# crowsonkb/k-diffusion

Hardware: AMD Instinct MI355X
Metric: images/sec, 256x256 image_transformer_v2, 50-step DPM++2M (whole job) (higher is better)
Workload: dtype f32

## Files before the change

### include/kdiff_hip.h

```cpp
#ifndef KDIFF_HIP_H
#define KDIFF_HIP_H

#ifdef __cplusplus
extern "C" {
#endif

#define KD_OK 0
#define KD_EINVAL (-1)
#define KD_ELAUNCH (-2)

int kd_version(void);
const char* kd_last_error(void);
int kd_set_option(const char* name, int value);
int kd_get_option(const char* name, int dflt);

enum { KD_A_PLAIN = 0, KD_A_MERGE2x2 = 1, KD_A_PATCH_NCHW = 2 };
enum { KD_PREC_EXACT = 0, KD_PREC_SPLIT3 = 1,
       KD_PREC_BF16 = 2  };
enum { KD_EPI_STORE = 0, KD_EPI_RESIDUAL = 1, KD_EPI_GEGLU = 2, KD_EPI_SPLIT_LERP = 3, KD_EPI_UNPATCH_NCHW = 4,
       KD_EPI_QKV = 5  };

typedef struct {
  int M, N, K;
  int a_mode, epi;
// ... 14 lines not shown
  const float* fac;
  int precision;
  const void* Wp;
  int n_heads;
  const float* qk_scale;
  const float* rope_cos;
  const float* rope_sin;
  int qkv_packed;
  const float* rope_pos;
  const float* rope_freq;
  int a_split, c_split;
  const void* A_lo;
  void* C_lo;
  int per_row;
} KdGemm;

int kd_gemm_f32(const KdGemm* desc, void* stream);

int kd_gemm_bf16(const KdGemm* desc, void* stream);
long long kd_packed_weight_bytes_bf16(int N, int K, int geglu);
int kd_pack_weight_bf16(const float* W, void* out, int N, int K, int geglu, void* stream);

typedef struct KdFfn {
  const void* x;
  void* out;
  const float* scale;
  int scale_stride, rows_per_sample;
  float eps;
  const void* Wp_up;
  const void* Wp_down;
  int M, K, d_ff;
  const void* attn;
  const void* Wp_out;
} KdFfn;
int kd_ffn_bf16_supported(int M, int K, int d_ff);
int kd_ffn_bf16(const KdFfn* desc, void* stream);
int kd_ffn_f32_supported(int M, int K, int d_ff);
int kd_ffn_f32(const KdFfn* desc, void* stream);

long long kd_packed_weight_bytes(int N, int K, int geglu);
int kd_pack_weight_bf16x3(const float* W, void* out, int N, int K, int geglu, void* stream);

int kd_norm_split_f32(const float* x, const float* scale, int scale_stride, int rows_per_sample, void* hi, void* lo, int M, int K,
                      float eps, void* stream);

int kd_rmsnorm_f32(const float* x, const float* scale, float* y, int rows, int d, float eps, void* stream);

int kd_fourier_sigma_f32(const float* sigma, const float* weight, float* ff, int batch, int half, void* stream);
int kd_fourier_f32(const float* in, const float* weight, float* ff, int batch, int in_dim, int half, void* stream);
int kd_cond_sum_f32(float* out, const float* a, const float* b, int b_rows, const float* emb,
                    const long long* ids, const float* c, int batch, int d, void* stream);

int kd_qk_prep_f32(float* qkv, const float* scale_h, const float* cos_t, const float* sin_t,
                   int batch, int tokens_per_sample, int nh, float eps, void* stream);

int kd_attn_global_f32(const float* qkv, float* out, int batch, int T, int nh,
                       int prep, const float* scale_h, const float* cos_t, const float* sin_t, float eps,
                       int precision, void* stream);

int kd_attn_window_f32(const float* qkv, float* out, int batch, int H, int W, int nh, int ws, int shift,
                       int prep, const float* scale_h, const float* cos_t, const float* sin_t, float eps,
                       int precision, void* stream);

int kd_attn_na2d_f32(const float* qkv, float* out, int batch, int H, int W, int nh, int ks,
                     int prep, const float* scale_h, const float* cos_t, const float* sin_t, float eps,
                     int precision, void* stream);

int kd_attn_global_bf16(const void* qkv, void* out, int batch, int T, int nh, void* stream);
int kd_attn_window_bf16(const void* qkv, void* out, int batch, int H, int W, int nh, int ws, int shift, void* stream);
int kd_attn_na2d_bf16(const void* qkv, void* out, int batch, int H, int W, int nh, int ks, void* stream);
// ... 97 lines not shown
```

### k-diffusion_amd/_native.py

```python
import ctypes as C
import os

_HERE = os.path.dirname(os.path.abspath(__file__))
LIB_PATH = os.environ.get("KDIFF_HIP_LIB") or os.path.join(_HERE, "csrc", "libkdiff_hip.so")

A_PLAIN, A_MERGE2x2, A_PATCH_NCHW = 0, 1, 2
EPI_STORE, EPI_RESIDUAL, EPI_GEGLU, EPI_SPLIT_LERP, EPI_UNPATCH_NCHW, EPI_QKV = 0, 1, 2, 3, 4, 5
PREC_EXACT, PREC_SPLIT3, PREC_BF16 = 0, 1, 2
PC_ONE, PC_SKIP, PC_OUT, PC_IN = 0, 1, 2, 3
PREC_FP8 = 3
_MODES = {"exact": PREC_EXACT, "split3": PREC_SPLIT3, "bf16": PREC_BF16, "fp8": PREC_FP8}


def default_precision():
    mode = os.environ.get("KDIFF_GEMM", "split3").lower()
    if mode not in _MODES:
        raise ValueError(f"KDIFF_GEMM={mode!r}: expected one of {sorted(_MODES)}")
    return _MODES[mode]


def kernel_precision():
    p = default_precision()
    return PREC_BF16 if p == PREC_FP8 else p


def precision_name(p):
    return {v: k for k, v in _MODES.items()}[p]
(STEP_EULER, STEP_HEUN_PRED, STEP_HEUN_CORR, STEP_DPMPP_2M1, STEP_DPMPP_2M2, STEP_ADD_NOISE, STEP_LERP2, STEP_AXPY,
 STEP_EULER_FROM, STEP_AXPBY, STEP_ADD_DIFF, STEP_TO_D) = range(12)


class KdGemm(C.Structure):
    _fields_ = [
        ("M", C.c_int), ("N", C.c_int), ("K", C.c_int),
        ("a_mode", C.c_int), ("epi", C.c_int), ("norm", C.c_int),
        ("rows_per_sample", C.c_int), ("scale_stride", C.c_int),
        ("gh", C.c_int), ("gw", C.c_int), ("ph", C.c_int), ("pw", C.c_int), ("chan", C.c_int),
        ("eps", C.c_float), ("out_add", C.c_float), ("sigma_data", C.c_float),
        ("A", C.c_void_p), ("W", C.c_void_p), ("C", C.c_void_p), ("R", C.c_void_p),
        ("scale", C.c_void_p), ("sigma", C.c_void_p), ("fac", C.c_void_p),
        ("precision", C.c_int), ("Wp", C.c_void_p),
        ("n_heads", C.c_int), ("qk_scale", C.c_void_p), ("rope_cos", C.c_void_p), ("rope_sin", C.c_void_p),
        ("qkv_packed", C.c_int), ("rope_pos", C.c_void_p), ("rope_freq", C.c_void_p),
        ("a_split", C.c_int), ("c_split", C.c_int), ("A_lo", C.c_void_p), ("C_lo", C.c_void_p),
        ("per_row", C.c_int),
    ]


class KdFfn(C.Structure):
    _fields_ = [
        ("x", C.c_void_p), ("out", C.c_void_p), ("scale", C.c_void_p),
        ("scale_stride", C.c_int), ("rows_per_sample", C.c_int), ("eps", C.c_float),
        ("Wp_up", C.c_void_p), ("Wp_down", C.c_void_p),
        ("M", C.c_int), ("K", C.c_int), ("d_ff", C.c_int),
        ("attn", C.c_void_p), ("Wp_out", C.c_void_p),
    ]


class KdCall(C.Structure):
    _fields_ = [("op", C.c_int), ("f", C.c_float), ("p", C.c_void_p * 5), ("i", C.c_int * 8)]


_vp, _i, _f, _ll, _d = C.c_void_p, C.c_int, C.c_float, C.c_longlong, C.c_double

SIGNATURES = {
    "kd_version": [],
    "kd_last_error": [],
    "kd_set_option": [C.c_char_p, _i],
    "kd_get_option": [C.c_char_p, _i],
    "kd_gemm_f32": [C.POINTER(KdGemm), _vp],
    "kd_gemm_bf16": [C.POINTER(KdGemm), _vp],
    "kd_packed_weight_bytes_bf16": [_i, _i, _i],
    "kd_pack_weight_bf16": [_vp, _vp, _i, _i, _i, _vp],
    "kd_ffn_bf16_supported": [_i, _i, _i],
    "kd_ffn_bf16": [_vp, _vp],
    "kd_ffn_f32_supported": [_i, _i, _i],
    "kd_ffn_f32": [_vp, _vp],
    "kd_attn_global_bf16": [_vp, _vp, _i, _i, _i, _vp],
    "kd_attn_window_bf16": [_vp, _vp, _i, _i, _i, _i, _i, _i, _vp],
    "kd_attn_na2d_bf16": [_vp, _vp, _i, _i, _i, _i, _i, _vp],
    "kd_attn_block_bf16_supported": [_i, _i, _i],
    "kd_attn_block_bf16": [C.POINTER(KdGemm), _vp],
    "kd_proj_block_bf16_supported": [_i, _i, _i, _i],
    "kd_proj_block_bf16": [C.POINTER(KdGemm), _vp],
    "kd_packed_weight_bytes_mx8": [_i, _i, _i],
    "kd_pack_weight_mx8": [_vp, _vp, _i, _i, _i, _vp],
    "kd_gemm_mx8_supported": [_i, _i, _i, _i, _i],
    "kd_gemm_mx8": [C.POINTER(KdGemm), _vp],
    "kd_packed_weight_bytes": [_i, _i, _i],
    "kd_pack_weight_bf16x3": [_vp, _vp, _i, _i, _i, _vp],
    "kd_rmsnorm_f32": [_vp, _vp, _vp, _i, _i, _f, _vp],
    "kd_fourier_sigma_f32": [_vp, _vp, _vp, _i, _i, _vp],
    "kd_fourier_f32": [_vp, _vp, _vp, _i, _i, _i, _vp],
    "kd_cond_sum_f32": [_vp, _vp, _vp, _i, _vp, _vp, _vp, _i, _i, _vp],
    "kd_qk_prep_f32": [_vp, _vp, _vp, _vp, _i, _i, _i, _f, _vp],
    "kd_attn_global_f32": [_vp, _vp, _i, _i, _i, _i, _vp, _vp, _vp, _f, _i, _vp],
    "kd_attn_window_f32": [_vp, _vp, _i, _i, _i, _i, _i, _i, _i, _vp, _vp, _vp, _f, _i, _vp],
    "kd_attn_na2d_f32": [_vp, _vp, _i, _i, _i, _i, _i, _i, _vp, _vp, _vp, _f, _i, _vp],
    "kd_sampler_step_f32": [_i, _vp, _vp, _vp, _vp, _vp, _f, _f, _f, _f, _ll, _vp],
    "kd_precond_in_f32": [_vp, _vp, _vp, _f, _i, _ll, _vp],
    "kd_precond_out_f32": [_vp, _vp, _vp, _vp, _f, _i, _ll, _vp],
    "kd_rows_affine_f32": [_vp, _vp, _vp, _vp, _vp, _i, _ll, _vp],
    "kd_sigma_to_t_f32": [_vp, _vp, _vp, _i, _i, _i, _vp],
    "kd_t_to_sigma_f32": [_vp, _vp, _vp, _i, _i, _vp],
    "kd_dpm_eps_f32": [_vp, _vp, _vp, _f, _ll, _vp],
    "kd_dpm_combine_f32": [_vp, _vp, _vp, _vp, _f, _f, _ll, _vp],
    "kd_dpm_error_partials": [],
    "kd_dpm_error_f32": [_vp, _vp, _vp, _f, _f, _ll, _vp, _vp],
    "kd_brownian_f32": [_vp, _vp, _i, _ll, _d, _d, _d, _d, _f, _i, _vp],
# ... 151 lines not shown
```

### k-diffusion_amd/csrc/common.cpp

```cpp
#include "kd_common.h"
#include <atomic>
#include <climits>
#include <mutex>

namespace kd {

static thread_local char g_err[512] = "";
char* err_buf() { return g_err; }

int fail(int code, const char* fmt, ...) {
  va_list ap;
  va_start(ap, fmt);
  vsnprintf(g_err, sizeof(g_err), fmt, ap);
  va_end(ap);
  return code;
}

static std::atomic<bool> g_prof{false};
static std::mutex g_rec_mutex;
static std::vector<ProfRec> g_recs;

bool prof_on() { return g_prof.load(std::memory_order_relaxed); }

static unsigned g_gen = 0;
// ... 11 lines not shown

void prof_end(ProfTicket t, hipStream_t s) {
  std::lock_guard<std::mutex> lock(g_rec_mutex);
  if (t.gen == g_gen && t.idx >= 0 && t.idx < (int)g_recs.size()) (void)hipEventRecord(g_recs[t.idx].e1, s);
}

}

namespace kd {
int cu_count() {
  static std::atomic<int> cache[64];
  int dev = 0;
  (void)hipGetDevice(&dev);
  if (dev < 0 || dev >= 64) dev = 0;
  int n = cache[dev].load(std::memory_order_relaxed);
  if (n <= 0) {
    if (hipDeviceGetAttribute(&n, hipDeviceAttributeMultiprocessorCount, dev) != hipSuccess || n <= 0) n = 256;
    cache[dev].store(n, std::memory_order_relaxed);
  }
  return n;
}
}

using namespace kd;

namespace kd {
namespace {
struct Opt { const char* name; std::atomic<int> value; std::atomic<bool> set; };
Opt g_opts[] = {{"skinny", {0}, {false}}, {"astat", {0}, {false}}, {"ksplit", {0}, {false}}, {"astat_max_k", {0}, {false}}, {"astat_waves", {0}, {false}},
                {"astat_storewait", {0}, {false}}, {"gemm_debug", {0}, {false}}, {"bf16_fast", {0}, {false}}, {"wstat", {0}, {false}},
                {"wstat_waves", {0}, {false}}, {"wstat_max_slices", {0}, {false}}, {"wstat_prefetch", {0}, {false}}, {"astat_bf16", {0}, {false}},
                {"astat_splits", {0}, {false}}, {"tiled_bm", {0}, {false}}, {"attn_global_qw", {0}, {false}},
                {"patch_fast", {0}, {false}}, {"ffn_fused", {0}, {false}}, {"ffn_fused_256", {0}, {false}}, {"astat_rows", {0}, {false}}, {"tiled_deep", {0}, {false}}, {"code_warm", {0}, {false}}, {"ffn_variant", {0}, {false}},
                {"x3", {0}, {false}}, {"x3_splits", {0}, {false}}, {"ffn_x3", {0}, {false}}, {"ffn_x3_half", {0}, {false}}, {"x3_res", {0}, {false}}, {"attn_x3", {0}, {false}}, {"x3_half", {0}, {false}}, {"x3r", {0}, {false}}, {"x3_unpatch", {0}, {false}}, {"x3r_lw", {0}, {false}}, {"x3r_split", {0}, {false}}, {"tiled_lw", {0}, {false}}, {"x3_min_rows", {0}, {false}}, {"x3r_min_rows", {0}, {false}}, {"ffn_x3_min_panels_256", {0}, {false}}, {"x3s_max_rows", {0}, {false}}, {"x3s_max_wgs", {0}, {false}}, {"x3s_scale_lds", {0}, {false}}, {"b16s_max_rows", {0}, {false}}, {"b16s_max_wgs", {0}, {false}}, {"ffn_bf16_min_rows", {0}, {false}}, {"x3s_trace", {0}, {false}}, {"attn_block_bf16", {0}, {false}}, {"proj_block_bf16", {0}, {false}}, {"mx8", {0}, {false}}, {"mx8_splits", {0}, {false}}, {"mx8_min_rows", {0}, {false}}};
constexpr int N_OPTS = sizeof(g_opts) / sizeof(g_opts[0]);
}
int option_index(const char* name) {
  for (int i = 0; i < N_OPTS; ++i)
    if (!strcmp(g_opts[i].name, name)) return i;
  return -1;
}
int option_at(int idx, int dflt) {
  if (idx < 0) return dflt;
  return g_opts[idx].set.load(std::memory_order_relaxed) ? g_opts[idx].value.load(std::memory_order_relaxed) : dflt;
}
}

extern "C" int kd_set_option(const char* name, int value) {
  if (!name) return fail(KD_EINVAL, "kd_set_option: null name");
  const int i = option_index(name);
  if (i < 0) return fail(KD_EINVAL, "kd_set_option: unknown option '%s'", name);
  if (value == INT_MIN) {
    g_opts[i].set.store(false, std::memory_order_relaxed);
    return KD_OK;
  }
  g_opts[i].value.store(value, std::memory_order_relaxed);
  g_opts[i].set.store(true, std::memory_order_relaxed);
  return KD_OK;
}
extern "C" int kd_get_option(const char* name, int dflt) { return name ? option_at(option_index(name), dflt) : dflt; }

extern "C" int kd_version(void) { return 200; }
extern "C" const char* kd_last_error(void) { return err_buf(); }

extern "C" int kd_prof_enable(int on) { g_prof.store(on != 0, std::memory_order_relaxed); return KD_OK; }
extern "C" int kd_prof_count(void) {
  std::lock_guard<std::mutex> lock(g_rec_mutex);
// ... 71 lines not shown
```

### k-diffusion_amd/csrc/ffn_x3.hip

```cpp
#include "x3_common.h"

namespace kd {
namespace x3 {

struct FArgs3 {
  const float* X; float* Y;
  const char* Wu; const char* Wd;
  const float* scale; int scale_stride, rows_per_sample; float eps;
  int M, d_ff, n_tiles;
  int warm;
  unsigned long long* clk;
  const float* Att; const char* Wo;
};

template <int IDX>
__device__ __forceinline__ void mfma_acc_ag(const bf16x8 w, const bf16x8 h) {
  asm volatile("v_mfma_f32_32x32x16_bf16 a[%c2:%c3], %0, %1, a[%c2:%c3]" :: "v"(w), "v"(h), "i"(IDX), "i"(IDX + 15) : KD_AGPR_ALL);
}
template <int IDX>
__device__ __forceinline__ void areg_zero16() {
  static_for<16>([&](auto i_) { asm volatile("v_accvgpr_write_b32 a[%c0], 0" :: "i"(IDX + decltype(i_)::value) : KD_AGPR_ALL); });
}
template <int IDX>
__device__ __forceinline__ f32x4 areg_read4() {
  f32x4 v;
  asm volatile("v_accvgpr_read_b32 %0, a[%c4]\n\tv_accvgpr_read_b32 %1, a[%c5]\n\tv_accvgpr_read_b32 %2, a[%c6]\n\tv_accvgpr_read_b32 %3, a[%c7]"
               : "=v"(v[0]), "=v"(v[1]), "=v"(v[2]), "=v"(v[3]) : "i"(IDX), "i"(IDX + 1), "i"(IDX + 2), "i"(IDX + 3));
  return v;
}

template <int IDX, int BIDX>
__device__ __forceinline__ void mfma_acc_aa(const bf16x8 w) {
  asm volatile("v_mfma_f32_32x32x16_bf16 a[%c1:%c2], %0, a[%c3:%c4], a[%c1:%c2]" :: "v"(w), "i"(IDX), "i"(IDX + 15), "i"(BIDX), "i"(BIDX + 3) : KD_AGPR_ALL);
}

template <int NC , bool OUTP = false >
__global__ __launch_bounds__(256, 1) void ffn_x3_kernel(const FArgs3 p) {
  static_assert(!OUTP || NC == 16, "fused out projection: width 256 here, width 128 in ffn_x3h_kernel");
  constexpr int K = NC * 16, NKU = NC / 2;
  constexpr int NOB = K / 32, NKD = 2 * (K / 128);
  constexpr int UNIT = NKU + NKD;
  constexpr int NSTG = 8, PDIST = NSTG - 1, PB = 4;
  constexpr bool AG = NC >= 16;
  constexpr int AO = AG ? 8 * NC : 0;
  constexpr int WAREA = (NSTG / 4) * STG;
// ... 395 lines not shown
    static_for<4>([&](auto g_) { blk[decltype(g_)::value] = areg_read4<AO + 16 * ob + 4 * decltype(g_)::value>(); });
#pragma unroll
    for (int hb = 0; hb < 2; ++hb) {
      const f32x4 (&skip)[2] = skip_all[ob][hb];
#pragma unroll
      for (int gg = 0; gg < 2; ++gg)
        *reinterpret_cast<f32x4*>(strip + l31 * 64 + (((2 * gg + lh) ^ ((l31 >> 2) & 1)) << 4)) = blk[2 * hb + gg];
#pragma unroll
      for (int it = 0; it < 2; ++it) {
        const int r16 = 16 * it + (lane >> 2), c = lane & 3;
        const f32x4 o = *reinterpret_cast<const f32x4*>(strip + r16 * 64 + ((c ^ ((r16 >> 2) & 1)) << 4));
        if (st_ok[it]) st16(st_row[it] + 32 * ob + 16 * hb, f32x4(o + skip[it]));
      }
    }
  });
  if (probe) { p.clk[2] = __builtin_amdgcn_s_memtime(); p.clk[3] = __builtin_amdgcn_s_memrealtime(); p.clk[7] = (unsigned long long)total; }
  wg_stamp_end(wgs);
}


template <int IDX>
__device__ __forceinline__ void mfma_acc_ag_lo(const bf16x8 w, const bf16x8 h) {
  asm volatile("v_mfma_f32_32x32x16_bf16 a[%c2:%c3], %0, %1, a[%c2:%c3]" :: "v"(w), "v"(h), "i"(IDX), "i"(IDX + 15) : KD_AGPR_LO128);
}
template <int IDX, int BIDX>
__device__ __forceinline__ void mfma_acc_aa_lo(const bf16x8 w) {
  asm volatile("v_mfma_f32_32x32x16_bf16 a[%c1:%c2], %0, a[%c3:%c4], a[%c1:%c2]" :: "v"(w), "i"(IDX), "i"(IDX + 15), "i"(BIDX), "i"(BIDX + 3) : KD_AGPR_LO128);
}
template <int IDX>
__device__ __forceinline__ void areg_zero16_lo() {
  static_for<16>([&](auto i_) { asm volatile("v_accvgpr_write_b32 a[%c0], 0" :: "i"(IDX + decltype(i_)::value) : KD_AGPR_LO128); });
}

template <bool OUTP>
__global__ __launch_bounds__(256, 2) void ffn_x3h_kernel(const FArgs3 p) {
  constexpr int NC = 8, K = 128, NOB = 4;
  constexpr int NSTG = 4, PDIST = NSTG - 1, PB = 4, UNIT = 3;
  constexpr int AO = 64;
  constexpr int CPR = K / 4, PIECES = 32 * CPR / 64, SCL = 1024, SUB = 8192, HALF = 4096;
  extern __shared__ __attribute__((aligned(16))) char smem[];
  const int tid = threadIdx.x, lane = tid & 63, l31 = lane & 31, lh = lane >> 5;
  const int wid = __builtin_amdgcn_readfirstlane(tid >> 6);
  const auto warm = code_warm_begin<16 * 1024>((int)blockIdx.x < p.warm && tid < 64);
  const int m0 = blockIdx.x * 128;
  const int T2 = 2 * p.n_tiles;
  const bool probe = p.clk && blockIdx.x == (gridDim.x * 5) / 8 && tid == 0;
  if (probe) { p.clk[0] = __builtin_amdgcn_s_memtime(); p.clk[1] = __builtin_amdgcn_s_memrealtime(); }
  const WgStamp wgs = wg_stamp_begin(p.clk);

  auto issue_rel = [&](int th, auto off_, int j) {
    constexpr int off = decltype(off_)::value, u = off % UNIT;
    const int tt = min(th + off / UNIT, T2 - 1);
    char* slot = smem + ((th * UNIT + off) % NSTG) * STG;
    const char* src;
    char* dst;
    if constexpr (u < 2) {
      src = p.Wu + ((size_t)(tt >> 1) * (NC / 2) + 2 * u + (j >> 1)) * STG + (j & 1) * IMG + (tt & 1) * HALF + wid * 1024 + lane * 16;
      dst = slot + (j >> 1) * SUB + (j & 1) * HALF + wid * 1024;
    } else {
      src = p.Wd + (size_t)tt * STG + wid * (PB * 1024) + j * 1024 + lane * 16;
      dst = slot + wid * (PB * 1024) + j * 1024;
    }
    __builtin_amdgcn_global_load_lds((const __attribute__((address_space(1))) void*)src, (__attribute__((address_space(3))) void*)dst, 16, 0, 0);
  };

  const int row = m0 + wid * 32 + l31;
  const bool ok = row < p.M;
// ... 328 lines not shown
    const int r = m0 + wid * 32 + 16 * it + (lane >> 2);
    st_ok[it] = r < p.M;
    st_row[it] = p.Y + (size_t)min(r, p.M - 1) * K + 4 * (lane & 3);
    sk_row[it] = p.X + (size_t)min(r, p.M - 1) * K + 4 * (lane & 3);
  }
  f32x4 skip_all[NOB][2][2];
#pragma unroll
  for (int ob = 0; ob < NOB; ++ob)
#pragma unroll
    for (int hb = 0; hb < 2; ++hb)
#pragma unroll
      for (int it = 0; it < 2; ++it)
        skip_all[ob][hb][it] = OUTP ? f32x4{0.f, 0.f, 0.f, 0.f} : *reinterpret_cast<const f32x4*>(sk_row[it] + 32 * ob + 16 * hb);
  __builtin_amdgcn_sched_barrier(0);
  asm volatile("s_waitcnt vmcnt(0)\n\ts_nop 15\n\ts_nop 3" ::: "memory");
  static_for<NOB>([&](auto ob_) {
    constexpr int ob = decltype(ob_)::value;
    f32x4 blk[4];
    static_for<4>([&](auto g_) { blk[decltype(g_)::value] = areg_read4<AO + 16 * ob + 4 * decltype(g_)::value>(); });
#pragma unroll
    for (int hb = 0; hb < 2; ++hb) {
      const f32x4 (&skip)[2] = skip_all[ob][hb];
#pragma unroll
      for (int gg = 0; gg < 2; ++gg)
        *reinterpret_cast<f32x4*>(strip + l31 * 64 + (((2 * gg + lh) ^ ((l31 >> 2) & 1)) << 4)) = blk[2 * hb + gg];
#pragma unroll
      for (int it = 0; it < 2; ++it) {
        const int r16 = 16 * it + (lane >> 2), c = lane & 3;
        const f32x4 o = *reinterpret_cast<const f32x4*>(strip + r16 * 64 + ((c ^ ((r16 >> 2) & 1)) << 4));
        if (st_ok[it]) st16(st_row[it] + 32 * ob + 16 * hb, f32x4(o + skip[it]));
      }
    }
  });
  if (probe) { p.clk[2] = __builtin_amdgcn_s_memtime(); p.clk[3] = __builtin_amdgcn_s_memrealtime(); p.clk[7] = (unsigned long long)(T2 * UNIT); }
  wg_stamp_end(wgs);
}

extern unsigned long long* g_clk;

template <bool OUTP>
static int launch_ffn_half(const FArgs3& a, const char* nm, double flops, double bytes, hipStream_t s) {
  constexpr int LDS = 4 * STG + 4 * 1024 + 4 * 2048;
  auto kern = ffn_x3h_kernel<OUTP>;
  static LdsAttr attr_set;
  attr_set.ensure(reinterpret_cast<const void*>(kern), LDS);
  LaunchScope prof(nm, flops, bytes, s);
  hipLaunchKernelGGL(kern, dim3((unsigned)((a.M + 127) / 128)), dim3(256), LDS, s, a);
  return check_launch("kd_ffn_f32");
}

template <int NC, bool OUTP = false>
static int launch_ffn(const FArgs3& a, const char* nm, double flops, double bytes, hipStream_t s) {
  auto kern = ffn_x3_kernel<NC, OUTP>;
  constexpr int K = NC * 16;
  constexpr int LDS = 8 * STG + 4 * (K * 4 < 1024 ? 1024 : K * 4) + 4 * 2048;
  static LdsAttr attr_set;
  attr_set.ensure(reinterpret_cast<const void*>(kern), LDS);
  LaunchScope prof(nm, flops, bytes, s);
  hipLaunchKernelGGL(kern, dim3((unsigned)((a.M + 127) / 128)), dim3(256), LDS, s, a);
  return check_launch("kd_ffn_f32");
}

}
}

using namespace kd;

extern "C" int kd_ffn_f32_supported(int M, int K, int d_ff) {
  if (!option("ffn_x3", 1)) return 0;
  if (!((K == 128 || K == 256) && d_ff > 0 && d_ff % 64 == 0)) return 0;
  if (K == 128) return M >= 2048;
  int dev = 0, cus = 256;
  (void)hipGetDevice(&dev);
  if (hipDeviceGetAttribute(&cus, hipDeviceAttributeMultiprocessorCount, dev) != hipSuccess || cus <= 0) cus = 256;
  const int need = option("ffn_x3_min_panels_256", cus - cus / 8);
  return (M + 127) / 128 >= need;
}

extern "C" int kd_ffn_f32(const KdFfn* dp, void* stream) {
  if (!dp) return fail(KD_EINVAL, "kd_ffn_f32: null descriptor");
  const KdFfn& d = *dp;
  if (!d.x || !d.out || !d.scale || !d.Wp_up || !d.Wp_down) return fail(KD_EINVAL, "kd_ffn_f32: null x / out / scale / Wp_up / Wp_down");
  if ((d.K != 128 && d.K != 256) || d.d_ff <= 0 || (d.d_ff & 63) || d.M <= 0) return fail(KD_EINVAL, "kd_ffn_f32: K must be 128 or 256, d_ff a multiple of 64 (K=%d d_ff=%d)", d.K, d.d_ff);
  if (d.rows_per_sample <= 0 || (d.scale_stride & 3)) return fail(KD_EINVAL, "kd_ffn_f32: rows_per_sample > 0, scale_stride %% 4 == 0");
  x3::FArgs3 a{};
  a.X = reinterpret_cast<const float*>(d.x); a.Y = reinterpret_cast<float*>(d.out);
  a.Wu = reinterpret_cast<const char*>(d.Wp_up); a.Wd = reinterpret_cast<const char*>(d.Wp_down);
  a.scale = d.scale; a.scale_stride = d.scale_stride; a.rows_per_sample = d.rows_per_sample; a.eps = d.eps;
  a.M = d.M; a.d_ff = d.d_ff; a.n_tiles = d.d_ff / 64;
  a.warm = option("code_warm", KD_CODE_WARM_DEFAULT);
  a.clk = x3::g_clk;
  const double flops = 2.0 * d.M * 3.0 * d.d_ff * d.K;
  const double bytes = 4.0 * (2.0 * d.M * d.K + 3.0 * d.d_ff * d.K);
  char nm[96] = "ffn_x3";
  if (prof_on()) snprintf(nm, sizeof(nm), "ffn_x3 M=%d K=%d d_ff=%d", d.M, d.K, d.d_ff);
  if (d.attn) {
    if (!d.Wp_out) return fail(KD_EINVAL, "kd_ffn_f32: attn without Wp_out");
    a.Att = reinterpret_cast<const float*>(d.attn); a.Wo = reinterpret_cast<const char*>(d.Wp_out);
    const double fl2 = flops + 2.0 * d.M * d.K * d.K, by2 = 4.0 * (3.0 * d.M * d.K + 3.0 * d.d_ff * d.K + (double)d.K * d.K);
    if (prof_on()) snprintf(nm, sizeof(nm), "ffn_x3+out M=%d K=%d d_ff=%d", d.M, d.K, d.d_ff);
    if (d.K == 128) return x3::launch_ffn_half<true>(a, nm, fl2, by2, (hipStream_t)stream);
    return x3::launch_ffn<16, true>(a, nm, fl2, by2, (hipStream_t)stream);
  }
  if (d.K == 128 && option("ffn_x3_half", 1)) return x3::launch_ffn_half<false>(a, nm, flops, bytes, (hipStream_t)stream);
  if (d.K == 128) return x3::launch_ffn<8>(a, nm, flops, bytes, (hipStream_t)stream);
  return x3::launch_ffn<16>(a, nm, flops, bytes, (hipStream_t)stream);
}

KD_TEXT_PAD(ffn_x3)
```

### k-diffusion_amd/models/image_transformer_v2.py

```python
import ctypes as C
import gc
import itertools
import operator
import weakref
import os
import math
from dataclasses import dataclass
from typing import NamedTuple, Optional, Union

import torch
from torch import nn

from .. import _native as nat
from .. import ops
from . import axial_rope

D_HEAD = 64
SCHEDULE_TABLE_MAX_BYTES = 1 << 30
SCHEDULES_KEPT = 4
SCHEDULE_CHAINS_KEPT = 2
DERIVED_KEPT = 1024
MAX_PLANS = 16
PLAN_SWITCHES = (("KDIFF_ATTN_BLOCK", "1"), ("KDIFF_PROJ_BLOCK", "1"), ("KDIFF_FFN_OUT", "all"), ("KDIFF_RUN_LIST", "1"))
CLASS_IDS_KEPT = 4
# ... 323 lines not shown
        self.out_shape = (B, m.out_channels, H, W)
        self.class_checked = {}

        self.sigma = torch.empty(B, **f32)
        self.sigma_ptr = self.sigma.data_ptr()
        self.xs = xs = [torch.empty(B, gh, gw, lv.width, **act) for (gh, gw), lv in zip(grids, levels)]
        self.toks = toks = [B * gh * gw for gh, gw in grids]
        self.qkv = torch.empty(max(t * 3 * lv.width for t, lv in zip(toks, levels)), **act)
        self.att = torch.empty(max(t * lv.width for t, lv in zip(toks, levels)), **act)
        self.hid = torch.empty(max(t * lv.d_ff for t, lv in zip(toks, levels)), **act)
        wide = [t * lv.width for t, lv in zip(toks, levels) if _prepass(mode, lv.width)]
        self.xn = torch.empty(max(wide), **f32) if wide else None
        norm_mods = m._ada_norm_modules()
        self.table_offsets, total = {}, 0
        for name, mod in norm_mods:
            self.table_offsets[name] = 4 * total
            total += mod.linear.weight.shape[0]
        wcat = m._packed.get("ada_norm_wcat")
        if wcat is None or wcat.device != device:
            wcat = m._packed["ada_norm_wcat"] = torch.cat([mod.linear.weight.detach() for _, mod in norm_mods], dim=0).contiguous()
        self.wcat = wcat
        self.scales = [torch.empty(B, total, **f32), torch.empty(B, total, **f32)]
        self.norm_descs = []
        self.last_buf, self.prefetched = 1, None
        self.side_stream = torch.cuda.Stream(device=device)
        self.main_entry = torch.cuda.Event()
        self.schedules, self.schedule_chains = [], {}
        self.scale_width = total
        self.step_chain = self.build_cond(B)

        L = self.launches
        self.d_patch_in = self._gemm(L, "patch_in", None, m.patch_in.proj.weight, xs[0], toks[0], levels[0].width, m.in_channels * ph * pw,
                                     a_mode=nat.A_PATCH_NCHW, grid=grids[0], patch=(ph, pw, m.in_channels))
        for st in hourglass(m):
            li = st.level
            if st.kind == "layer":
                self._add_layer(li, st.prefix, st.module, st.index)
            elif st.kind == "merge":
                self._gemm(L, f"merges.{li}", xs[li], m.merges[li].proj.weight, xs[li + 1], toks[li + 1], levels[li + 1].width,
                           4 * levels[li].width, a_mode=nat.A_MERGE2x2, grid=grids[li + 1])
            else:
                self._gemm(L, f"splits.{li}", xs[li + 1], m.splits[li].proj.weight, xs[li], toks[li + 1], 4 * levels[li].width,
                           levels[li + 1].width, epi=nat.EPI_SPLIT_LERP, residual=xs[li], fac=m.splits[li].fac, grid=grids[li + 1])
        self.d_patch_out = self._gemm(L, "patch_out", xs[0], m.patch_out.proj.weight, None, toks[0], m.out_channels * ph * pw,
                                      levels[0].width, epi=nat.EPI_UNPATCH_NCHW, norm_scale=m.out_norm.scale, scale_stride=0,
                                      rows_per_sample=grids[0][0] * grids[0][1], grid=grids[0], patch=(ph, pw, m.out_channels))
        self._encode_launches()

    def _gemm(self, launches, what, A, Wt, Cc, M, N, K, cond=False, table=None, entry=None, mx8=False, **kw):
        precision = self.cond_precision if cond else self.precision
        if table is not None:
            kw.update(scale_ptr=0, scale_stride=self.scale_width)
        d = ops.gemm(A, Wt, Cc, M=M, N=N, K=K, precision=precision, per_row=cond, mx8=mx8, launch=False, pack=self.model._packed_image, **kw)
        if table is not None:
            self.norm_descs.append((d, self.table_offsets[table]))
        launches.append(_Launch(entry or ops._gemm_entry(precision, mx8), (d,), what + ("(mx8)" if mx8 else "")))
        return d

    def _norm_split(self, launches, table, x, T, d, rps):
        ref = _ScaleRef()
        self.norm_descs.append((ref, self.table_offsets[table]))
        planes = self.xn.view(torch.bfloat16)
        hi, lo = planes[:T * d], planes[T * d:2 * T * d]
        launches.append(_Launch("kd_norm_split_f32", (_ptr(x), ref, self.scale_width, rps, _ptr(hi), _ptr(lo), T, d, 1e-6), table + " (split)"))
        return hi, lo

    def build_cond(self, rows):
        m, f32 = self.model, dict(device=self.device, dtype=torch.float32)
        mw, mdff = m.mapping_spec.width, m.mapping_spec.d_ff
# ... 40 lines not shown

    def _qk(self, li, sa, nh):
        m = self.model
        if self.precision == nat.PREC_BF16:
            cos_t, sin_t = m._rope(li, self.grids, sa, self.device, revs=True)
        else:
            cos_t, sin_t = m._rope(li, self.grids, sa, self.device)
        self.keep += [cos_t, sin_t]
        qk = (sa.scale, cos_t, sin_t, nh)
        if self.precision == nat.PREC_SPLIT3:
            pos_t, freq_t = m._rope(li, self.grids, sa, self.device, revs=True)
            self.keep += [pos_t, freq_t]
            qk += (pos_t, freq_t)
        return qk

    def _add_layer(self, li, prefix, mod, index):
        L, lv, (gh, gw), T = self.launches, self.levels[li], self.grids[li], self.toks[li]
        d, d_ff, x, rps = lv.width, lv.d_ff, self.xs[li], gh * gw
        spec = lv.self_attn
        nh = d // spec.d_head if hasattr(mod, "self_attn") else 0
        kind, core, params = attn_geometry(spec, index) if nh else (None, None, ())
        r = route_layer(self.lib, self.mode, self.B, T, rps, d, d_ff, nh, kind, self.switches)
        split3 = self.precision == nat.PREC_SPLIT3
        if nh:
            sa, norm = mod.self_attn, prefix + "self_attn.norm"
            q = dict(epi=nat.EPI_QKV, rows_per_sample=rps, qk=self._qk(li, sa, nh), qkv_packed=split3)
            if r.qkv == "attn_block":
                self._gemm(L, prefix + "attn_block", x, sa.qkv_proj.weight, self.att, T, 3 * d, d, table=norm, entry="kd_attn_block_bf16", **q)
            elif r.qkv == "split":
                planes = self._norm_split(L, norm, x, T, d, rps)
                self._gemm(L, prefix + "qkv_proj", None, sa.qkv_proj.weight, self.qkv, T, 3 * d, d, a_planes=planes, **q)
            elif r.qkv == "proj_block":
                self._gemm(L, prefix + "qkv_proj(block)", x, sa.qkv_proj.weight, self.qkv, T, 3 * d, d, table=norm, entry="kd_proj_block_bf16", **q)
            else:
                self._gemm(L, prefix + "qkv_proj", x, sa.qkv_proj.weight, self.qkv, T, 3 * d, d, table=norm, mx8=r.qkv == "mx8", **q)
            if r.core is not None:
                geo = ((rps, nh) if kind == "global" else (gh, gw, nh)) + params
                prep = () if r.core.endswith("_bf16") else (2 if split3 else 0, None, None, None, C.c_float(1e-6), self.precision)
                L.append(_Launch(r.core, (_ptr(self.qkv), _ptr(self.att), self.B, *geo, *prep), prefix + core))
            if not r.fuse_out:
                self._gemm(L, prefix + "out_proj", self.att, sa.out_proj.weight, x, T, d, d, epi=nat.EPI_RESIDUAL, residual=x)
        norm, w_up, w_down = prefix + "ff.norm", mod.ff.up_proj.weight, mod.ff.down_proj.weight
        if r.ff != "pair":
            fd = ops.ffn(x, None, w_up, w_down, out=x, scale_stride=self.scale_width, rows_per_sample=rps, attn=self.att if r.fuse_out else None,
                         w_out=mod.self_attn.out_proj.weight if r.fuse_out else None, launch=False, pack=self.model._packed_image)
            self.norm_descs.append((fd, self.table_offsets[norm]))
            L.append(_Launch(r.ff, (fd,), prefix + "ff"))
            return
        hid8 = None
        if r.up == "split":
            planes = self._norm_split(L, norm, x, T, d, rps)
            self._gemm(L, prefix + "up_proj", None, w_up, self.hid, T, d_ff, d, epi=nat.EPI_GEGLU, a_planes=planes)
        else:
            if r.down_mx8:
                b = self.hid.view(torch.uint8)
                hid8 = (b[:T * d_ff], b[T * d_ff:T * d_ff + T * d_ff // 32])
            block = r.up == "proj_block"
            self._gemm(L, prefix + ("up_proj(block)" if block else "up_proj"), x, w_up, self.hid, T, d_ff, d, epi=nat.EPI_GEGLU, table=norm,
                       rows_per_sample=rps, mx8=r.up == "mx8", c_planes=hid8, entry="kd_proj_block_bf16" if block else None)
        if r.down_mx8:
            self._gemm(L, prefix + "down_proj", None, w_down, x, T, d, d_ff, epi=nat.EPI_RESIDUAL, residual=x, a_planes=hid8, mx8=True)
        else:
            self._gemm(L, prefix + "down_proj", self.hid, w_down, x, T, d, d_ff, epi=nat.EPI_RESIDUAL, residual=x)

    def run_cond(self, buf, stream):
        self.step_chain.run(self.scales[buf].data_ptr(), stream)

    def run(self, x, out, sigma_data, base):
        for d, off in self.norm_descs:
            d.scale = base + off
        pin, pout = self.d_patch_in, self.d_patch_out
        pin.A = x.data_ptr()
        pout.C = out.data_ptr()
        if sigma_data is None:
            pin.sigma, pout.sigma, pout.R = None, None, None
        else:
            sp = self.sigma_ptr
            pin.sigma, pout.sigma, pout.R = sp, sp, x.data_ptr()
            pin.sigma_data = pout.sigma_data = float(sigma_data)
        stream = C.c_void_p(torch.cuda.current_stream().cuda_stream)
        if self.calls is not None:
# ... 395 lines not shown
```

Baseline: 227.7.

## Fuse next layer's QKV projection into the tail of the fused f32 FFN kernel

Adds a QKV_NEXT variant of the two-workgroup split3 FFN kernel. After writing its FFN output rows, each workgroup computes the RMS norm, the split-bf16x3 QKV GEMM and the qk/RoPE prep for those same rows of the following layer, so that layer skips its separate qkv_proj launch. This removes a kernel launch and a global re-read of the activations. In exchange it adds LDS use and a long serial tail per workgroup, and it is gated by a heuristic that only enables it when splitting N across workgroups would not give better occupancy.

```diff
diff --git a/include/kdiff_hip.h b/include/kdiff_hip.h
--- a/include/kdiff_hip.h
+++ b/include/kdiff_hip.h
@@ -70,10 +70,12 @@
   int M, K, d_ff;
   const void* attn;
   const void* Wp_out;
+  const KdGemm* qkv_next;
 } KdFfn;
 int kd_ffn_bf16_supported(int M, int K, int d_ff);
 int kd_ffn_bf16(const KdFfn* desc, void* stream);
 int kd_ffn_f32_supported(int M, int K, int d_ff);
+int kd_ffn_f32_qkv_next_supported(int M, int K, int d_ff, int N, int n_heads);
 int kd_ffn_f32(const KdFfn* desc, void* stream);
 
 long long kd_packed_weight_bytes(int N, int K, int geglu);
diff --git a/k-diffusion_amd/_native.py b/k-diffusion_amd/_native.py
--- a/k-diffusion_amd/_native.py
+++ b/k-diffusion_amd/_native.py
@@ -54,6 +54,7 @@
         ("Wp_up", C.c_void_p), ("Wp_down", C.c_void_p),
         ("M", C.c_int), ("K", C.c_int), ("d_ff", C.c_int),
         ("attn", C.c_void_p), ("Wp_out", C.c_void_p),
+        ("qkv_next", C.c_void_p),
     ]
 
 
@@ -75,6 +76,7 @@
     "kd_ffn_bf16_supported": [_i, _i, _i],
     "kd_ffn_bf16": [_vp, _vp],
     "kd_ffn_f32_supported": [_i, _i, _i],
+    "kd_ffn_f32_qkv_next_supported": [_i, _i, _i, _i, _i],
     "kd_ffn_f32": [_vp, _vp],
     "kd_attn_global_bf16": [_vp, _vp, _i, _i, _i, _vp],
     "kd_attn_window_bf16": [_vp, _vp, _i, _i, _i, _i, _i, _i, _vp],
diff --git a/k-diffusion_amd/csrc/common.cpp b/k-diffusion_amd/csrc/common.cpp
--- a/k-diffusion_amd/csrc/common.cpp
+++ b/k-diffusion_amd/csrc/common.cpp
@@ -67,7 +67,7 @@
                 {"wstat_waves", {0}, {false}}, {"wstat_max_slices", {0}, {false}}, {"wstat_prefetch", {0}, {false}}, {"astat_bf16", {0}, {false}},
                 {"astat_splits", {0}, {false}}, {"tiled_bm", {0}, {false}}, {"attn_global_qw", {0}, {false}},
                 {"patch_fast", {0}, {false}}, {"ffn_fused", {0}, {false}}, {"ffn_fused_256", {0}, {false}}, {"astat_rows", {0}, {false}}, {"tiled_deep", {0}, {false}}, {"code_warm", {0}, {false}}, {"ffn_variant", {0}, {false}},
-                {"x3", {0}, {false}}, {"x3_splits", {0}, {false}}, {"ffn_x3", {0}, {false}}, {"ffn_x3_half", {0}, {false}}, {"x3_res", {0}, {false}}, {"attn_x3", {0}, {false}}, {"x3_half", {0}, {false}}, {"x3r", {0}, {false}}, {"x3_unpatch", {0}, {false}}, {"x3r_lw", {0}, {false}}, {"x3r_split", {0}, {false}}, {"tiled_lw", {0}, {false}}, {"x3_min_rows", {0}, {false}}, {"x3r_min_rows", {0}, {false}}, {"ffn_x3_min_panels_256", {0}, {false}}, {"x3s_max_rows", {0}, {false}}, {"x3s_max_wgs", {0}, {false}}, {"x3s_scale_lds", {0}, {false}}, {"b16s_max_rows", {0}, {false}}, {"b16s_max_wgs", {0}, {false}}, {"ffn_bf16_min_rows", {0}, {false}}, {"x3s_trace", {0}, {false}}, {"attn_block_bf16", {0}, {false}}, {"proj_block_bf16", {0}, {false}}, {"mx8", {0}, {false}}, {"mx8_splits", {0}, {false}}, {"mx8_min_rows", {0}, {false}}};
+                {"x3", {0}, {false}}, {"x3_splits", {0}, {false}}, {"ffn_x3", {0}, {false}}, {"ffn_qkv_next", {0}, {false}}, {"ffn_x3_half", {0}, {false}}, {"x3_res", {0}, {false}}, {"attn_x3", {0}, {false}}, {"x3_half", {0}, {false}}, {"x3r", {0}, {false}}, {"x3_unpatch", {0}, {false}}, {"x3r_lw", {0}, {false}}, {"x3r_split", {0}, {false}}, {"tiled_lw", {0}, {false}}, {"x3_min_rows", {0}, {false}}, {"x3r_min_rows", {0}, {false}}, {"ffn_x3_min_panels_256", {0}, {false}}, {"x3s_max_rows", {0}, {false}}, {"x3s_max_wgs", {0}, {false}}, {"x3s_scale_lds", {0}, {false}}, {"b16s_max_rows", {0}, {false}}, {"b16s_max_wgs", {0}, {false}}, {"ffn_bf16_min_rows", {0}, {false}}, {"x3s_trace", {0}, {false}}, {"attn_block_bf16", {0}, {false}}, {"proj_block_bf16", {0}, {false}}, {"mx8", {0}, {false}}, {"mx8_splits", {0}, {false}}, {"mx8_min_rows", {0}, {false}}};
 constexpr int N_OPTS = sizeof(g_opts) / sizeof(g_opts[0]);
 }
 int option_index(const char* name) {
diff --git a/k-diffusion_amd/csrc/ffn_x3.hip b/k-diffusion_amd/csrc/ffn_x3.hip
--- a/k-diffusion_amd/csrc/ffn_x3.hip
+++ b/k-diffusion_amd/csrc/ffn_x3.hip
@@ -2,6 +2,12 @@
 
 namespace kd {
 namespace x3 {
+
+struct QNext {
+  const char* Wp; float* C;
+  const float* scale; int scale_stride, rows_per_sample; float eps;
+  int n_tiles, n_heads; const float* qk_scale; const float* pos; const float* freq; int qkv_packed;
+};
 
 struct FArgs3 {
   const float* X; float* Y;
@@ -11,6 +17,7 @@
   int warm;
   unsigned long long* clk;
   const float* Att; const char* Wo;
+  QNext q;
 };
 
 template <int IDX>
@@ -472,7 +479,242 @@
   static_for<16>([&](auto i_) { asm volatile("v_accvgpr_write_b32 a[%c0], 0" :: "i"(IDX + decltype(i_)::value) : KD_AGPR_LO128); });
 }
 
-template <bool OUTP>
+template <int IDX>
+__device__ __forceinline__ f32x16 areg_read16() {
+  f32x16 v;
+  static_for<4>([&](auto g_) {
+    constexpr int g = decltype(g_)::value;
+    const f32x4 t = areg_read4<IDX + 4 * g>();
+#pragma unroll
+    for (int e = 0; e < 4; ++e) v[4 * g + e] = t[e];
+  });
+  return v;
+}
+
+__device__ __forceinline__ void qkv_next_rows(const QNext& q, const float* X, const int M, const int m0) {
+  constexpr int NC = 8, K = 128, NK = NC / 2, NSTG = 4, PDIST = NSTG - 1, PB = 4, NCOL = 128, NST = 16, SCL = 1024;
+  constexpr int CPR = K / 4, PIECES = 32 * CPR / 64, AO = 64;
+  extern __shared__ __attribute__((aligned(16))) char smem[];
+  int tid = threadIdx.x;
+  asm volatile("" : "+v"(tid));
+  const int lane = tid & 63, l31 = lane & 31, lh = lane >> 5;
+  const int wid = __builtin_amdgcn_readfirstlane(tid >> 6);
+  const int n_tiles = q.n_tiles, total = n_tiles * NK;
+  const char* wp = q.Wp + wid * (PB * 1024) + lane * 16;
+  auto issue_piece = [&](int s_, int j) {
+    const int s = min(s_, total - 1);
+    const char* src = wp + (size_t)s * STG;
+    char* dst = smem + (s_ % NSTG) * STG + wid * (PB * 1024);
+    __builtin_amdgcn_global_load_lds((const __attribute__((address_space(1))) void*)(src + j * 1024),
+                                     (__attribute__((address_space(3))) void*)(dst + j * 1024), 16, 0, 0);
+  };
+  auto issue = [&](int s_) {
+#pragma unroll
+    for (int j = 0; j < PB; ++j) issue_piece(s_, j);
+  };
+
+  const int row = m0 + wid * 32 + l31;
+  const int rowc = row < M ? row : M - 1;
+  float rs0;
+  {
+    char* stage = smem + wid * STG;
+    char* scl = smem + NSTG * STG + wid * SCL;
+    const int r_first = min(m0 + wid * 32, M - 1), r_last = min(m0 + wid * 32 + 31, M - 1);
+    const bool uni = q.scale_stride == 0 || r_first / q.rows_per_sample == r_last / q.rows_per_sample;
+    if (uni) {
+      const char* ssrc = reinterpret_cast<const char*>(q.scale + (size_t)(r_first / q.rows_per_sample) * q.scale_stride);
+      __builtin_amdgcn_global_load_lds((const __attribute__((address_space(1))) void*)(ssrc + (lane * 16) % (K * 4)),
+                                       (__attribute__((address_space(3))) void*)scl, 16, 0, 0);
+    }
+    const float* sp = q.scale + (size_t)(rowc / q.rows_per_sample) * q.scale_stride + 8 * lh;
+    const float* spl = reinterpret_cast<const float*>(scl) + 8 * lh;
+    float ssq = 0.f;
+#pragma unroll
+    for (int i = 0; i < PIECES; ++i) {
+      const int ci = i * 64 + lane, rr = ci / CPR, qs = ci % CPR;
+      const int grow = min(m0 + wid * 32 + rr, M - 1);
+      const char* src = reinterpret_cast<const char*>(X + (size_t)grow * K) + ((qs ^ (rr & 15)) << 4);
+      __builtin_amdgcn_global_load_lds((const __attribute__((address_space(1))) void*)src,
+                                       (__attribute__((address_space(3))) void*)(stage + i * 1024), 16, 0, 0);
+    }
+    asm volatile("s_waitcnt vmcnt(0)" ::: "memory");
+    const char* rowp = stage + l31 * (K * 4);
+    static_for<NC / 4>([&](auto c4_) {
+      constexpr int c0 = 4 * decltype(c4_)::value;
+      f32x4 x0[4], x1[4], s0[4], s1[4];
+#pragma unroll
+      for (int u = 0; u < 4; ++u) {
+        const int qq = 4 * (c0 + u) + 2 * lh;
+        x0[u] = *reinterpret_cast<const f32x4*>(rowp + ((qq ^ (l31 & 15)) << 4));
+        x1[u] = *reinterpret_cast<const f32x4*>(rowp + (((qq + 1) ^ (l31 & 15)) << 4));
+        if (uni) {
+          s0[u] = *reinterpret_cast<const f32x4*>(spl + 16 * (c0 + u));
+          s1[u] = *reinterpret_cast<const f32x4*>(spl + 16 * (c0 + u) + 4);
+        } else {
+          s0[u] = *reinterpret_cast<const f32x4*>(sp + 16 * (c0 + u));
+          s1[u] = *reinterpret_cast<const f32x4*>(sp + 16 * (c0 + u) + 4);
+        }
+      }
+      __builtin_amdgcn_sched_barrier(0);
+      static_for<4>([&](auto u_) {
+        constexpr int u = decltype(u_)::value;
+#pragma unroll
+        for (int e = 0; e < 4; ++e) ssq = fmaf(x0[u][e], x0[u][e], fmaf(x1[u][e], x1[u][e], ssq));
+        u32x4 hi, lo;
+        split8(x0[u] * s0[u], x1[u] * s1[u], hi, lo);
+        areg_write4_lo<8 * (c0 + u)>(hi);
+        areg_write4_lo<8 * (c0 + u) + 4>(lo);
+      });
+      __builtin_amdgcn_sched_barrier(0);
+    });
+    ssq += __shfl_xor(ssq, 32, 64);
+    rs0 = rsqrtf(ssq / (float)K + q.eps);
+  }
+  float* qk_tab = reinterpret_cast<float*>(smem + NSTG * STG + 4 * SCL + 4 * 2048);
+  if (tid < q.n_heads * 8) qk_tab[tid] = q.freq[tid];
+  if (tid < q.n_heads) qk_tab[128 + tid] = sqrtf(q.qk_scale[tid]);
+  float py0, px0;
+  {
+    const int tok = rowc % q.rows_per_sample;
+    py0 = q.pos[2 * tok];
+    px0 = q.pos[2 * tok + 1];
+    asm volatile("" : "+v"(py0), "+v"(px0));
+  }
+  float* park = reinterpret_cast<float*>(smem + NSTG * STG + wid * SCL) + lane;
+  park[0] = rs0;
+  park[64] = py0;
+  park[128] = px0;
+  static_for<4>([&](auto j_) { areg_zero16_lo<AO + 16 * decltype(j_)::value>(); });
+  asm volatile("s_waitcnt vmcnt(0) lgkmcnt(0)" ::: "memory");
+  KD_BARRIER();
+  const bool full_panel = m0 + 128 <= M;
+#pragma unroll
+  for (int s = 0; s < PDIST; ++s) issue(s);
+
+  const int o0 = swz64(l31, lh), o1 = swz64(l31, 2 + lh);
+  char* strip = smem + NSTG * STG + 4 * SCL + wid * 2048;
+  const char* qkc = smem + NSTG * STG + 4 * SCL + 4 * 2048;
+  const int N = n_tiles * NCOL;
+  float* st_row[2];
+  bool st_ok[2];
+#pragma unroll
+  for (int it = 0; it < 2; ++it) {
+    const int r = m0 + wid * 32 + 16 * it + (lane >> 2);
+    st_ok[it] = r < M;
+    st_row[it] = q.C + (size_t)min(r, M - 1) * N + 4 * (lane & 3);
+  }
+  bf16x8 wh[2][4], wl[2][4];
+  auto read_frags = [&](int slot, int h, bf16x8 (&fh)[4], bf16x8 (&fl)[4]) {
+    const char* st = smem + slot * STG + (h ? o1 : o0);
+#pragma unroll
+    for (int j = 0; j < 4; ++j) {
+      fh[j] = *reinterpret_cast<const bf16x8*>(st + j * 32 * 64);
+      fl[j] = *reinterpret_cast<const bf16x8*>(st + IMG + j * 32 * 64);
+    }
+  };
+  wait_vm(PB * (PDIST - 1));
+  KD_BARRIER();
+  read_frags(0, 0, wh[0], wl[0]);
+  asm volatile("s_nop 3" ::: "memory");
+
+  constexpr std::integral_constant<int, 0> I0{};
+  constexpr std::integral_constant<int, 1> I1{};
+  constexpr std::integral_constant<int, 2> I2{};
+  constexpr std::integral_constant<int, 3> I3{};
+  for (int nt = 0; nt < n_tiles; ++nt) {
+    static_for<NK>([&](auto ks_) {
+      constexpr int ks = decltype(ks_)::value;
+      const int s = nt * NK + ks;
+      auto mm = [&](auto b_, auto j_, bool w_lo, auto a_lo_) {
+        constexpr int b = decltype(b_)::value, j = decltype(j_)::value, al = decltype(a_lo_)::value, c = 2 * ks + b;
+        mfma_acc_aa_lo<AO + 16 * j, 8 * c + 4 * al>(w_lo ? wl[b][j] : wh[b][j]);
+      };
+      mm(I0, I0, true, I0);
+      __builtin_amdgcn_sched_barrier(0);
+      read_frags(ks % NSTG, 1, wh[1], wl[1]);
+      __builtin_amdgcn_sched_barrier(0);
+      mm(I0, I1, true, I0); mm(I0, I2, true, I0); mm(I0, I3, true, I0);
+      mm(I0, I0, false, I1); mm(I0, I1, false, I1); mm(I0, I2, false, I1); mm(I0, I3, false, I1);
+      mm(I0, I0, false, I0); mm(I0, I1, false, I0); mm(I0, I2, false, I0); mm(I0, I3, false, I0);
+      __builtin_amdgcn_sched_barrier(0);
+      {
+        int allow = PB * (PDIST - 2);
+        if (full_panel && nt > 0 && ks + 2 <= PDIST) allow += NST;
+        wait_vm(allow);
+        KD_BARRIER();
+      }
+      mm(I1, I0, true, I0);
+      __builtin_amdgcn_sched_barrier(0);
+      read_frags((ks + 1) % NSTG, 0, wh[0], wl[0]);
+      __builtin_amdgcn_sched_barrier(0);
+      mm(I1, I1, true, I0); mm(I1, I2, true, I0);
+      issue_piece(s + PDIST, 0);
+      __builtin_amdgcn_sched_barrier(0);
+      mm(I1, I3, true, I0); mm(I1, I0, false, I1); mm(I1, I1, false, I1);
+      issue_piece(s + PDIST, 1);
+      __builtin_amdgcn_sched_barrier(0);
+      mm(I1, I2, false, I1); mm(I1, I3, false, I1); mm(I1, I0, false, I0);
+      issue_piece(s + PDIST, 2);
+      __builtin_amdgcn_sched_barrier(0);
+      mm(I1, I1, false, I0); mm(I1, I2, false, I0);
+      issue_piece(s + PDIST, 3);
+      mm(I1, I3, false, I0);
+      __builtin_amdgcn_sched_barrier(0);
+    });
+    asm volatile("s_nop 15\n\ts_nop 3" ::: "memory");
+
+    const int n0 = nt * NCOL;
+    auto store_block = [&](const f32x4 (&v)[4], int col) {
+#pragma unroll
+      for (int hb = 0; hb < 2; ++hb) {
+#pragma unroll
+        for (int gg = 0; gg < 2; ++gg)
+          *reinterpret_cast<f32x4*>(strip + l31 * 64 + (((2 * gg + lh) ^ ((l31 >> 2) & 1)) << 4)) = v[2 * hb + gg];
+#pragma unroll
+        for (int it = 0; it < 2; ++it) {
+          const int r16 = 16 * it + (lane >> 2), c = lane & 3;
+          const f32x4 o = *reinterpret_cast<const f32x4*>(strip + r16 * 64 + ((c ^ ((r16 >> 2) & 1)) << 4));
+          if (st_ok[it]) st16(st_row[it] + col + 16 * hb, o);
+        }
+      }
+    };
+    const float rs = park[0], py = park[64], px = park[128];
+    static_for<2>([&](auto vv_) {
+      constexpr int vv = decltype(vv_)::value;
+      const int vec = (n0 >> 6) + vv;
+      const int which = vec >= 2 * q.n_heads ? 2 : (vec >= q.n_heads ? 1 : 0), head = vec - which * q.n_heads;
+      f32x16 a0 = areg_read16<AO + 32 * vv>();
+      f32x16 a1 = areg_read16<AO + 32 * vv + 16>();
+      if (which < 2) {
+        const f32x4 fv = *reinterpret_cast<const f32x4*>(qkc + (head * 8 + 4 * lh) * 4);
+        const float qsc = *reinterpret_cast<const float*>(qkc + 512 + head * 4);
+        const float fr[4] = {fv[0], fv[1], fv[2], fv[3]};
+        b16::qk_prep_blocks(a0, a1, rs, qsc, q.eps, py, px, fr);
+      } else {
+#pragma unroll
+        for (int r = 0; r < 16; ++r) { a0[r] *= rs; a1[r] *= rs; }
+      }
+#pragma unroll
+      for (int jj = 0; jj < 2; ++jj) {
+        f32x4 blk[4];
+        const f32x16& a = jj ? a1 : a0;
+        if (q.qkv_packed) {
+#pragma unroll
+          for (int g = 0; g < 4; ++g) blk[g] = pack_split4(f32x4{a[4 * g], a[4 * g + 1], a[4 * g + 2], a[4 * g + 3]});
+        } else {
+#pragma unroll
+          for (int g = 0; g < 4; ++g) blk[g] = f32x4{a[4 * g], a[4 * g + 1], a[4 * g + 2], a[4 * g + 3]};
+        }
+        store_block(blk, n0 + 64 * vv + 32 * jj);
+      }
+    });
+    static_for<4>([&](auto j_) { areg_zero16_lo<AO + 16 * decltype(j_)::value>(); });
+    asm volatile("s_nop 3" ::: "memory");
+  }
+  asm volatile("s_waitcnt vmcnt(0)" ::: "memory");
+}
+
+template <bool OUTP, bool QKV_NEXT = false>
 __global__ __launch_bounds__(256, 2) void ffn_x3h_kernel(const FArgs3 p) {
   constexpr int NC = 8, K = 128, NOB = 4;
   constexpr int NSTG = 4, PDIST = NSTG - 1, PB = 4, UNIT = 3;
@@ -867,16 +1109,21 @@
       }
     }
   });
+  if constexpr (QKV_NEXT) {
+    asm volatile("s_waitcnt vmcnt(0)" ::: "memory");
+    KD_BARRIER();
+    qkv_next_rows(p.q, p.Y, p.M, m0);
+  }
   if (probe) { p.clk[2] = __builtin_amdgcn_s_memtime(); p.clk[3] = __builtin_amdgcn_s_memrealtime(); p.clk[7] = (unsigned long long)(T2 * UNIT); }
   wg_stamp_end(wgs);
 }
 
 extern unsigned long long* g_clk;
 
-template <bool OUTP>
+template <bool OUTP, bool QKV_NEXT = false>
 static int launch_ffn_half(const FArgs3& a, const char* nm, double flops, double bytes, hipStream_t s) {
-  constexpr int LDS = 4 * STG + 4 * 1024 + 4 * 2048;
-  auto kern = ffn_x3h_kernel<OUTP>;
+  constexpr int LDS = 4 * STG + 4 * 1024 + 4 * 2048 + (QKV_NEXT ? 1024 : 0);
+  auto kern = ffn_x3h_kernel<OUTP, QKV_NEXT>;
   static LdsAttr attr_set;
   attr_set.ensure(reinterpret_cast<const void*>(kern), LDS);
   LaunchScope prof(nm, flops, bytes, s);
@@ -910,6 +1157,16 @@
   if (hipDeviceGetAttribute(&cus, hipDeviceAttributeMultiprocessorCount, dev) != hipSuccess || cus <= 0) cus = 256;
   const int need = option("ffn_x3_min_panels_256", cus - cus / 8);
   return (M + 127) / 128 >= need;
+}
+
+extern "C" int kd_ffn_f32_qkv_next_supported(int M, int K, int d_ff, int N, int n_heads) {
+  if (!option("ffn_qkv_next", 1) || K != 128 || !option("ffn_x3_half", 1) || !kd_ffn_f32_supported(M, K, d_ff)) return 0;
+  if (!option("x3", 1) || M < option("x3_min_rows", 512) || option("x3_splits", 0) || n_heads <= 0 || n_heads > 16 || N != 3 * 64 * n_heads || N % 128) return 0;
+  const int n_tiles = N / 128;
+  const long panels = (M + 127) / 128, slots = 2L * cu_count();
+  for (int sp = 2; sp <= n_tiles; ++sp)
+    if (n_tiles % sp == 0 && ((panels * sp + slots - 1) / slots) * (1 + n_tiles / sp) < ((panels + slots - 1) / slots) * (1 + n_tiles)) return 0;
+  return 1;
 }
 
 extern "C" int kd_ffn_f32(const KdFfn* dp, void* stream) {
@@ -929,6 +1186,26 @@
   const double bytes = 4.0 * (2.0 * d.M * d.K + 3.0 * d.d_ff * d.K);
   char nm[96] = "ffn_x3";
   if (prof_on()) snprintf(nm, sizeof(nm), "ffn_x3 M=%d K=%d d_ff=%d", d.M, d.K, d.d_ff);
+  if (d.qkv_next) {
+    const KdGemm& g = *d.qkv_next;
+    if (d.K != 128 || !option("ffn_x3_half", 1) || g.epi != KD_EPI_QKV || g.precision != KD_PREC_SPLIT3 || !g.norm || g.a_mode != KD_A_PLAIN
+        || g.a_split || g.c_split || g.A != d.out || g.M != d.M || g.K != d.K || g.n_heads <= 0 || g.n_heads > 16 || g.N != 3 * 64 * g.n_heads
+        || (g.N & 127) || !g.Wp || !g.C || !g.scale || !g.qk_scale || !g.rope_pos || !g.rope_freq || g.rows_per_sample <= 0)
+      return fail(KD_EINVAL, "kd_ffn_f32: qkv_next needs K = 128 (two-workgroup kernel) and a split3 norm -> KD_EPI_QKV descriptor on out (N = 3 x 64 n_heads, n_heads <= 16)");
+    a.q.Wp = reinterpret_cast<const char*>(g.Wp); a.q.C = g.C;
+    a.q.scale = g.scale; a.q.scale_stride = g.scale_stride; a.q.rows_per_sample = g.rows_per_sample; a.q.eps = g.eps;
+    a.q.n_tiles = g.N / 128; a.q.n_heads = g.n_heads; a.q.qk_scale = g.qk_scale; a.q.pos = g.rope_pos; a.q.freq = g.rope_freq;
+    a.q.qkv_packed = g.qkv_packed;
+    const double fq = 2.0 * d.M * g.N * d.K, bq = 4.0 * ((double)g.N * d.K + (double)d.M * g.N);
+    if (prof_on()) snprintf(nm, sizeof(nm), "ffn_x3%s+qkv M=%d K=%d d_ff=%d", d.attn ? "+out" : "", d.M, d.K, d.d_ff);
+    if (d.attn) {
+      if (!d.Wp_out) return fail(KD_EINVAL, "kd_ffn_f32: attn without Wp_out");
+      a.Att = reinterpret_cast<const float*>(d.attn); a.Wo = reinterpret_cast<const char*>(d.Wp_out);
+      const double fl2 = flops + 2.0 * d.M * d.K * d.K, by2 = 4.0 * (3.0 * d.M * d.K + 3.0 * d.d_ff * d.K + (double)d.K * d.K);
+      return x3::launch_ffn_half<true, true>(a, nm, fl2 + fq, by2 + bq, (hipStream_t)stream);
+    }
+    return x3::launch_ffn_half<false, true>(a, nm, flops + fq, bytes + bq, (hipStream_t)stream);
+  }
   if (d.attn) {
     if (!d.Wp_out) return fail(KD_EINVAL, "kd_ffn_f32: attn without Wp_out");
     a.Att = reinterpret_cast<const float*>(d.attn); a.Wo = reinterpret_cast<const char*>(d.Wp_out);
diff --git a/k-diffusion_amd/models/image_transformer_v2.py b/k-diffusion_amd/models/image_transformer_v2.py
--- a/k-diffusion_amd/models/image_transformer_v2.py
+++ b/k-diffusion_amd/models/image_transformer_v2.py
@@ -379,9 +379,12 @@
         L = self.launches
         self.d_patch_in = self._gemm(L, "patch_in", None, m.patch_in.proj.weight, xs[0], toks[0], levels[0].width, m.in_channels * ph * pw,
                                      a_mode=nat.A_PATCH_NCHW, grid=grids[0], patch=(ph, pw, m.in_channels))
+        self.ffn_tail = None
         for st in hourglass(m):
             li = st.level
+            tail, self.ffn_tail = self.ffn_tail, None
             if st.kind == "layer":
+                self.ffn_tail = tail if tail is not None and tail[0] == li else None
                 self._add_layer(li, st.prefix, st.module, st.index)
             elif st.kind == "merge":
                 self._gemm(L, f"merges.{li}", xs[li], m.merges[li].proj.weight, xs[li + 1], toks[li + 1], levels[li + 1].width,
@@ -488,6 +491,10 @@
                 self._gemm(L, prefix + "qkv_proj", None, sa.qkv_proj.weight, self.qkv, T, 3 * d, d, a_planes=planes, **q)
             elif r.qkv == "proj_block":
                 self._gemm(L, prefix + "qkv_proj(block)", x, sa.qkv_proj.weight, self.qkv, T, 3 * d, d, table=norm, entry="kd_proj_block_bf16", **q)
+            elif r.qkv == "plain" and self.ffn_tail is not None and split3 and bool(self.lib.kd_ffn_f32_qkv_next_supported(T, d, d_ff, 3 * d, nh)):
+                qd = self._gemm([], prefix + "qkv_proj", x, sa.qkv_proj.weight, self.qkv, T, 3 * d, d, table=norm, **q)
+                self.keep.append(qd)
+                self.ffn_tail[1].qkv_next = C.addressof(qd)
             else:
                 self._gemm(L, prefix + "qkv_proj", x, sa.qkv_proj.weight, self.qkv, T, 3 * d, d, table=norm, mx8=r.qkv == "mx8", **q)
             if r.core is not None:
@@ -502,7 +509,9 @@
                          w_out=mod.self_attn.out_proj.weight if r.fuse_out else None, launch=False, pack=self.model._packed_image)
             self.norm_descs.append((fd, self.table_offsets[norm]))
             L.append(_Launch(r.ff, (fd,), prefix + "ff"))
+            self.ffn_tail = (li, fd) if r.ff == "kd_ffn_f32" else None
             return
+        self.ffn_tail = None
         hid8 = None
         if r.up == "split":
             planes = self._norm_split(L, norm, x, T, d, rps)
```

Result: no change. 227.8, median of 6 (+0.1%).
